# ml4ai/mliis

Hardware: AMD Instinct MI355X
Metric: inner-loop images/sec (EfficientLab-6-3, 224x224, 5-shot) (higher is better)
Workload: dtype f32 (the long-K decoder convs and their filter gradients with every operand split exactly into three bf16 terms on the matrix cores, 6 term products, f32 accumulate: fp32-equivalent products; everything else the fp32 instruction)

## Files before the change

include/mliis_hip.h:

```cpp
#ifndef MLIIS_HIP_H
#define MLIIS_HIP_H

#include <stddef.h>
#include <stdint.h>

#ifdef __cplusplus
extern "C" {
#endif

#ifndef __HIP__
typedef struct ihipStream_t* hipStream_t;
#endif

#if defined(__GNUC__) || defined(__clang__)
#pragma GCC visibility push(default)
#endif

#define MLIIS_OK 0
#define MLIIS_ERR_ARG (-1)
#define MLIIS_ERR_UNSUPPORTED (-2)
#define MLIIS_ERR_ALIGN (-3)
#define MLIIS_ERR_LAUNCH (-4)
#define MLIIS_ERR_WORKSPACE (-5)

// ... 76 lines not shown
int mliis_conv2d_fwd_bnin_ok(int Nimg, int H, int W, int Cin, int Cout);
int mliis_conv2d_fwd_bnin(const float* z, int ldz, const float* bn_part, int bn_nblk, float eps, float momentum, float* mean, float* rstd,
                          float* moving_mean, float* moving_var, const float* gamma, const float* beta, const float* img_scale,
                          const float* res, int ldr, float* a_out, int lda_out, const float* wt, float* y, int ldy, int Nimg, int H, int W,
                          int Cin, int Cout, float* stats_part, int stats_swish, int* stats_nblk, int precision, float fp8_act_scale,
                          const float* fp8_w_amax, int y_dtype, hipStream_t stream);
int mliis_transpose_weights(const float* src, float* dst, const int* desc, int ndesc, long long total_tiles, float* amax, hipStream_t stream);
int mliis_weight_shadows(const float* src, float* dst, const int* desc, int ndesc, long long total_tiles, float* amax, void* x3_images,
                         const long long* x3_desc, int x3_ndesc, int x3_blocks, hipStream_t stream);
int mliis_weight_shadows_rng(const float* src, float* dst, const int* desc, int ndesc, long long total_tiles, float* amax, void* x3_images,
                             const long long* x3_desc, int x3_ndesc, int x3_blocks, unsigned* rng_state, int njobs, float* const* outs,
                             const long long* numels, const float* keep, const float* const* keeps, const int* row_len, const int* floor_form,
                             hipStream_t stream);
int mliis_conv2d_bwd_data(const float* dy, int lddy, const float* w, float* dx, int lddx, int Nimg, int H, int W, int Cin_total,
                          int ci_begin, int Cin_out, int Cout, int ksize, int dil, int accumulate, float* ws, size_t ws_floats,
                          int precision, int dy_dtype, int dx_dtype, hipStream_t stream);
int mliis_conv2d_bwd_data_bn(const float* dy, int lddy, const float* w, float* dx, int lddx, int Nimg, int H, int W, int Cin_total,
                             int ci_begin, int Cin_out, int Cout, int ksize, int dil, int accumulate, float* ws, size_t ws_floats,
                             int precision, const float* bn_x, int bn_ldx, const float* bn_mean, const float* bn_rstd,
                             const float* bn_img_scale, float* part, size_t part_floats, int* nblk, int dy_dtype, int dx_dtype, hipStream_t stream);
int mliis_conv2d_bwd_data_gate(const float* dy, int lddy, const float* w, float* dx, int lddx, int Nimg, int H, int W, int Cin_total,
                               int ci_begin, int Cin_out, int Cout, int ksize, int dil, float* ws, size_t ws_floats, int precision,
                               const float* gate_x, int gate_ldx, float* part, size_t part_floats, int* groups, int dy_dtype, int dx_dtype, hipStream_t stream);
size_t mliis_x3_image_bytes(int Cred, int Nout, int ksize);
int mliis_x3_image_blocks(int Cred, int Nout, int ksize);
int mliis_x3_pack_weights(const float* theta, void* images, const long long* desc, int ndesc, int total_blocks, hipStream_t stream);
size_t mliis_conv2d_x3_workspace_floats(int Nimg, int H, int W, int Cred, int Nout, int ksize);
int mliis_conv2d_x3_plan(int Nimg, int H, int W, int Cred, int Nout, int ksize, int* plan);
int mliis_conv2d_fwd_x3(const float* x, int ldx, const void* image, size_t image_bytes, const float* bias, const float* border_bias, float* y, int ldy, int Nimg,
                        int H, int W, int Cin, int Cout, int ksize, int dil, int accumulate, float* stats_part, int stats_swish,
                        int* stats_nblk, float* ws, size_t ws_floats, hipStream_t stream);
int mliis_conv2d_bwd_data_x3(const float* dy, int lddy, const void* image, size_t image_bytes, float* dx, int lddx, int Nimg, int H, int W, int Cin_out, int Cout,
                             int ksize, int dil, int accumulate, float* ws, size_t ws_floats, hipStream_t stream);
size_t mliis_conv2d_bwd_filter_workspace_floats(int Nimg, int H, int W, int Cin, int Cout, int ksize);
int mliis_conv2d_bwd_filter(const float* x, int ldx, const float* x_scale, const float* dy, int lddy, float* dw, int Nimg, int H, int W,
                            int Cin_total, int ci_begin, int Cin, int Cout, int ksize, int dil, int accumulate, float* ws,
                            size_t ws_floats, int precision, hipStream_t stream);
int mliis_conv2d_bwd_filter_plan(int Nimg, int H, int W, int Cin, int Cout, int ksize, int* plan);
int mliis_conv2d_bwd_filter_batched(const long long* desc, int nprob, int blocks, int tmf, int nt, int has_scale, int precision,
                                    hipStream_t stream);

size_t mliis_rsd_concat_pool_floats(int N, int H, int W, int C);
int mliis_rsd_concat_pool(const float* deep, int ld_deep, int Hi, int Wi, int Cd, const float* skip, int ld_skip, int Cs, float* cat, int ldcat,
                          int N, int H, int W, float* pool_part, size_t pool_part_floats, int* chunks, hipStream_t stream);
int mliis_rsd_pool_fwd(const float* pool_part, int chunks, float scale, float* pool_out, const float* w, float* border_bias, int N, int Cp,
                       int Cin_total, int c_begin, int Co, hipStream_t stream);
// ... 111 lines not shown
```

mliis_amd/csrc/conv_gemm_kernels.hpp:

```cpp
#pragma once
#include <stdlib.h>

#include <type_traits>

#include "bn_fold.hpp"
#include "common.hpp"

namespace mliis {

typedef float f32x4 __attribute__((ext_vector_type(4)));

struct ConvGemmParams {
  const float* A;
  int lda;
  int Nimg, H, W;
  int C;
  int ntaps, dil, sign;
  const float* B;
  long long b_tap_stride;
  int ldb;
  int Nout;
  float* Cmat;
  int ldc;
  const float* bias;
// ... 1515 lines not shown
    case 5: L(T_, 5)  \
    case 6: L(T_, 6)  \
    case 7: L(T_, 7)  \
    default: L(T_, 8) \
  }
  if (f.tmf == 2) {
    ROW(2)
  } else {
    ROW(1)
  }
#undef ROW
#undef L
}

constexpr int kX3Block = 3072;
constexpr int kX3DescWords = 8;
__device__ __forceinline__ void x3_pack_block(const float* __restrict__ theta, char* __restrict__ images, const long long* __restrict__ desc,
                                              int ndesc, int b, int t) {
  int j = 0;
  for (int k = 1; k < ndesc; ++k)
    if (b >= (int)(desc[k * kX3DescWords + 6] >> 8)) j = k;
  const long long* d = desc + (long long)j * kX3DescWords;
  const float* w = theta + d[0];
  const int taps = (int)d[1], cin_total = (int)d[2], cout = (int)d[3], ci_begin = (int)d[4], cin = (int)d[5], mode = (int)(d[6] & 0xff);
  const int local = b - (int)(d[6] >> 8);
  const int nn = mode == 0 ? cout : cin, kc = mode == 0 ? cin : cout;
  const int ncol16 = (nn + 15) / 16;
  const int chunk = local / ncol16, c16 = local - chunk * ncol16;
  const int nl = t & 15, kq = t >> 4;
  const int n = c16 * 16 + nl;
  const int k = chunk * 32 + kq * 4;
  const int tap = k / kc, c = k - tap * kc;
  float4 v = f4zero();
  if (n < nn && tap < taps) {
    if (mode == 0) {
      const float* s = w + ((long long)tap * cin_total + ci_begin + c) * cout + n;
      v = make_float4(s[0], s[cout], s[2 * (long long)cout], s[3 * (long long)cout]);
    } else {
      v = ld4(w + ((long long)tap * cin_total + ci_begin + n) * cout + c);
    }
  }
  uint2 h, m, l;
  split3(v, h, m, l);
  char* dst = images + d[7] + (long long)local * kX3Block + (kq & 3) * 256 + nl * 16 + (kq >> 2) * 8;
  *reinterpret_cast<uint2*>(dst) = h;
  *reinterpret_cast<uint2*>(dst + 1024) = m;
  *reinterpret_cast<uint2*>(dst + 2048) = l;
}


void launch_gemm_bf16(const GemmPlan& g, const ConvGemmParams& p, hipStream_t stream);
void launch_gemm_sk_bf16(const GemmPlan& g, const ConvGemmParams& p, float* slab, hipStream_t stream);
void launch_gemm_fp8(const GemmPlan& g, const ConvGemmParams& p, hipStream_t stream);
bool launch_stream_lowp(int precision, int kc, int nt, dim3 grid, const ConvGemmParams& p, int row_groups, hipStream_t stream, bool ain = false);
bool launch_ksplit_lowp(int precision, int kc, int nt, dim3 grid, const ConvGemmParams& p, int row_groups, hipStream_t stream);
void launch_filter_bf16(const FilterPlan& f, const FilterGradParams& p, hipStream_t stream);
bool launch_filter_batched_bf16(int tmf, int nt, bool sc, const long long* desc, int nprob, int blocks, hipStream_t stream);
bool launch_filter_batched_x3(int nt, const long long* desc, int nprob, int blocks, int tile_ci, hipStream_t stream);

}
```

mliis_amd/csrc/conv_x3.hip:

```cpp
#include "conv_gemm_kernels.hpp"

namespace mliis {

constexpr int kX3BM = 256;
constexpr int kX3PF = 1;

__global__ __launch_bounds__(128) void x3_pack_k(const float* __restrict__ theta, char* __restrict__ images, const long long* __restrict__ desc,
                                                  int ndesc) {
  x3_pack_block(theta, images, desc, ndesc, blockIdx.x, threadIdx.x);
}

struct X3Params {
  ConvGemmParams g;
  const char* image;
  int ncol16;
};

template <int NT>
struct X3Sm {
  static constexpr int BN = 16 * NT;
  static constexpr int B_BYTES = NT * kX3Block;
  static constexpr int STAGES = 2;
  static constexpr int BYTES = STAGES * B_BYTES + 64;
};

template <int NT>
__device__ __forceinline__ void conv_x3_tile(const X3Params& q, char* __restrict__ sm, unsigned bx, int by, int it0, int it1,
                                             float* __restrict__ pdst) {
  constexpr int BN = 16 * NT;
  constexpr int B_BYTES = X3Sm<NT>::B_BYTES;
  constexpr int NB = (NT * 192 + 511) / 512;
  const ConvGemmParams& p = q.g;
  const int t = threadIdx.x, lane = t & 63;
  const int wave = __builtin_amdgcn_readfirstlane(t >> 6);
  const int l15 = lane & 15, g = lane >> 4;
  const long long M = (long long)p.Nimg * p.H * p.W;
  const long long m0 = (long long)bx * kX3BM;
  const int n0 = by * BN;
  const __amdgpu_buffer_rsrc_t rA = __builtin_amdgcn_make_buffer_rsrc((void*)p.A, 0, kBufRecords, 0x00020000);
  const __amdgpu_buffer_rsrc_t rB = __builtin_amdgcn_make_buffer_rsrc((void*)q.image, 0, kBufRecords, 0x00020000);

  const int wrow = wave * 32;
  unsigned a_row[2], a_taps[2];
#pragma unroll
  for (int rb = 0; rb < 2; ++rb) {
    const long long m = m0 + wrow + rb * 16 + l15;
    a_taps[rb] = 0;
    a_row[rb] = 0;
    if (m < M) {
      a_row[rb] = (unsigned)(m * p.lda * 4);
      if (p.ntaps > 1) {
        const int HWp = p.H * p.W;
        const int n = (int)(m / HWp);
        const int rem = (int)(m - (long long)n * HWp);
        const int h = rem / p.W, w_ = rem - h * p.W;
#pragma unroll
        for (int tp = 0; tp < 9; ++tp) {
          const int dh = (tp / 3 - 1) * p.dil * p.sign, dw = (tp % 3 - 1) * p.dil * p.sign;
          if ((unsigned)(h + dh) < (unsigned)p.H && (unsigned)(w_ + dw) < (unsigned)p.W) a_taps[rb] |= 1u << tp;
        }
      } else {
        a_taps[rb] = 1u;
      }
    }
  }
  int l_tap[2], l_c[2];
#pragma unroll
  for (int qd = 0; qd < 2; ++qd) {
    const int k0 = it0 * 32 + qd * 16 + g * 4;
    l_tap[qd] = k0 / p.C;
    l_c[qd] = k0 - l_tap[qd] * p.C;
  }
  int s_aleft = it1 - it0, s_bleft = it1 - it0;
  int ncol_here = q.ncol16 - by * NT;
  if (ncol_here > NT) ncol_here = NT;
  const unsigned b_lim = (unsigned)ncol_here * 192u;
  const unsigned b_step = (unsigned)q.ncol16 * kX3Block;
  unsigned b_voff[NB];
#pragma unroll
  for (int i = 0; i < NB; ++i) b_voff[i] = ((unsigned)t + 512u * i < b_lim) ? (unsigned)(by * NT) * kX3Block + ((unsigned)t + 512u * i) * 16u : kOob;
  unsigned s_boff = (unsigned)it0 * b_step;

  float4 ra[2][2];
  float4 ra2[2][2];
  u32x4 rbv[NB];
  const int tap_scale = p.dil * p.sign;
  auto load_a_into = [&](float4 (&ra)[2][2]) {
    const int adv = s_aleft > 1 ? 1 : 0;
    s_aleft -= adv;
#pragma unroll
    for (int qd = 0; qd < 2; ++qd) {
      const int tap = l_tap[qd];
      const int th = p.ntaps > 1 ? (tap * 11) >> 5 : 1, tw = p.ntaps > 1 ? tap - 3 * th : 1;
      const int dh = (th - 1) * tap_scale, dw = (tw - 1) * tap_scale;
      const unsigned koff = (unsigned)(((dh * p.W + dw) * p.lda + l_c[qd]) * 4);
      const unsigned tapbit = tap < p.ntaps ? 1u << tap : 0u;
#pragma unroll
      for (int rb = 0; rb < 2; ++rb) ra[rb][qd] = buf_ld4(rA, (a_taps[rb] & tapbit) != 0 ? a_row[rb] + koff : kOob);
      const int c_next = l_c[qd] + 32;
      const int wrap = c_next >= p.C ? 1 : 0;
      l_c[qd] = adv ? (wrap ? c_next - p.C : c_next) : l_c[qd];
      l_tap[qd] += adv & wrap;
    }
  };
  auto load_b_into = [&](u32x4 (&rbv)[NB]) {
#pragma unroll
    for (int i = 0; i < NB; ++i) {
      rbv[i] = __builtin_amdgcn_raw_buffer_load_b128(rB, (int)b_voff[i], (int)s_boff, 0);
    }
    const int adv = s_bleft > 1 ? 1 : 0;
    s_bleft -= adv;
    s_boff += adv ? b_step : 0u;
  };
  auto store_b_from = [&](char* buf, const u32x4 (&rbv)[NB]) {
#pragma unroll
    for (int i = 0; i < NB; ++i) {
      const int idx = t + 512 * i;
      char* d = (512 * (i + 1) <= NT * 192 || idx < NT * 192) ? buf + idx * 16 : sm + X3Sm<NT>::STAGES * B_BYTES + (t & 3) * 16;
      *reinterpret_cast<u32x4*>(d) = rbv[i];
// ... 79 lines not shown
      for (int rb = 0; rb < 2; ++rb) a3[pl][rb] = a3n[pl][rb];
  };
  {
    int it = 0;
    for (; it + 2 <= nper; it += 2) {
      chunk(sm, sm + B_BYTES, ra);
      chunk(sm + B_BYTES, sm, ra2);
    }
    if (it < nper) chunk(sm, sm + B_BYTES, ra);
  }
  asm volatile("s_waitcnt vmcnt(0)" ::: "memory");
#pragma unroll
  for (int rb = 0; rb < 2; ++rb)
#pragma unroll
    for (int r = 0; r < 4; ++r) {
      const int row = wrow + rb * 16 + g * 4 + r;
      if (m0 + row >= M) continue;
#pragma unroll
      for (int j = 0; j < NT; ++j)
        if (n0 + j * 16 + l15 < p.Nout) pdst[(long long)row * BN + j * 16 + l15] = acc[rb][j][r];
    }
}

template <int NT>
__global__ __launch_bounds__(512) void conv_x3_k(X3Params q, SkPlan k) {
  __shared__ __attribute__((aligned(16))) char sm[X3Sm<NT>::BYTES];
  constexpr int BN = 16 * NT;
#ifndef X3_NO_CLAIM
  asm volatile("v_mov_b32 v255, 0" ::: "v255");
#endif
  const int part = (int)xcd_remap(blockIdx.x, gridDim.x);
  int lo = part * k.ipp;
  const int total = k.rem * k.nchunks;
  int hi = lo + k.ipp;
  if (hi > total) hi = total;
#pragma unroll 1
  while (lo < hi) {
    const int rt = lo / k.nchunks, c0 = lo - rt * k.nchunks;
    int c1 = c0 + (hi - lo);
    if (c1 > k.nchunks) c1 = k.nchunks;
    const int first = (rt * k.nchunks) / k.ipp;
    float* dst = k.slab + ((long long)rt * k.smax + (part - first)) * (kX3BM * BN);
    conv_x3_tile<NT>(q, sm, rt / k.gy, rt % k.gy, c0, c1, dst);
    lo += c1 - c0;
    __syncthreads();
  }
}

constexpr int kX3Fix = 4;
template <int NT>
__global__ __launch_bounds__(1024) void x3_fixup_k(ConvGemmParams p, SkPlan k) {
  constexpr int BN = 16 * NT, QN = BN / 4;
  constexpr int QS = QN <= 32 ? 32 : 64;
  constexpr int RL = 1024 / QS;
  constexpr int RPT = kX3BM / kX3Fix / RL;
  __shared__ float4 red[2][RL][QS];
  const int t = threadIdx.x, q = t % QS, rl = t / QS;
  const int rt = blockIdx.x, sub = blockIdx.y;
  const unsigned tau = k.full + rt;
  const int bx = tau / k.gy, by = tau % k.gy;
  const long long M = (long long)p.Nimg * p.H * p.W;
  const int r0 = sub * (kX3BM / kX3Fix);
  const long long m0 = (long long)bx * kX3BM + r0;
  const int n = by * BN + q * 4;
  const bool cok = q < QN && n < p.Nout;
  const int first = (rt * k.nchunks) / k.ipp;
  int last = ((rt + 1) * k.nchunks - 1) / k.ipp;
  if (last > k.parts - 1) last = k.parts - 1;
  const int nslots = last - first + 1;
// ... 316 lines not shown
struct X3Plan {
  int nt, gx, gy, nchunks;
  int full, rem, parts, ipp, smax;
  size_t slab_floats() const { return (size_t)rem * smax * kX3BM * (16 * nt); }
};
constexpr int kX3MinPart = 4;

constexpr int kX3MaxNT = 9;
static int x3_pick_nt(int Nout) {
  int best = 1;
  double best_cost = 1e30;
  const int tiles = (Nout + 15) / 16;
  for (int nt = 1; nt <= kX3MaxNT; ++nt) {
    const int blocks = (tiles + nt - 1) / nt;
    const double cost = (double)(blocks * nt * 16) / (double)Nout * (1.0 + 0.08 * (8 - nt));
    if (cost < best_cost - 1e-9 || (cost < best_cost + 1e-9 && nt > best)) {
      best_cost = cost;
      best = nt;
    }
  }
  return best;
}

static inline int x3_chunks(int ntaps, int Cred) { return (ntaps * Cred + 31) / 32; }
static X3Plan x3_plan(long long M, int Nout, int ntaps, int Cred, int num_cus) {
  X3Plan g;
  g.nt = x3_pick_nt(Nout);
  g.gy = (Nout + g.nt * 16 - 1) / (g.nt * 16);
  g.gx = (int)((M + kX3BM - 1) / kX3BM);
  g.nchunks = x3_chunks(ntaps, Cred);
  const int slots = num_cus;
  while (g.nt > 2 && (long long)g.gx * g.gy * g.nchunks < (long long)slots * 2 * kX3MinPart) {
    g.nt = (g.nt + 1) / 2;
    g.gy = (Nout + g.nt * 16 - 1) / (g.nt * 16);
  }
  const long long tiles = (long long)g.gx * g.gy;
  g.full = 0;
  g.rem = (int)tiles;
  const long long total = tiles * g.nchunks;
  long long parts = slots;
  if (parts > 8LL * tiles) parts = 8LL * tiles;
  if (total / parts < kX3MinPart) parts = total / kX3MinPart;
  if (parts < 1) parts = 1;
  g.ipp = (int)((total + parts - 1) / parts);
  g.parts = (int)((total + g.ipp - 1) / g.ipp);
  g.smax = (g.nchunks + g.ipp - 1) / g.ipp + 1;
  return g;
}

static int g_x3_cus = 0;
static int x3_num_cus() {
  if (g_x3_cus == 0) {
    int dev = 0;
    hipDeviceProp_t prop;
    g_x3_cus = (hipGetDevice(&dev) == hipSuccess && hipGetDeviceProperties(&prop, dev) == hipSuccess && prop.multiProcessorCount > 0)
                   ? prop.multiProcessorCount
                   : 256;
  }
  return g_x3_cus;
}

static void x3_launch(const X3Plan& g, const X3Params& q_, float* slab, hipStream_t stream) {
  X3Params q = q_;
  const SkPlan k{g.full, g.rem, g.parts, g.ipp, g.nchunks, g.smax, g.gy, slab};
  dim3 grid(g.parts), block(512);
#define L(NT_)                                                                                  \
  hipLaunchKernelGGL((conv_x3_k<NT_>), grid, block, 0, stream, q, k);                           \
  hipLaunchKernelGGL((x3_fixup_k<NT_>), dim3(g.rem, kX3Fix), dim3(1024), 0, stream, q.g, k);    \
  break;
  switch (g.nt) {
    case 1: L(1)
    case 2: L(2)
    case 3: L(3)
    case 4: L(4)
    case 5: L(5)
    case 6: L(6)
    case 7: L(7)
    case 8: L(8)
    default: L(9)
  }
#undef L
}

static int x3_shape_check(const char* name, int Nimg, int H, int W, int Cred, int Nout, int ksize, int dil) {
  MLIIS_REQUIRE(Nimg > 0 && H > 0 && W > 0 && Cred >= 32 && Nout > 0, MLIIS_ERR_ARG, "%s: bad shape (the reduced channel count must be >= 32)", name);
  MLIIS_REQUIRE((Cred & 3) == 0 && (Nout & 3) == 0, MLIIS_ERR_ARG, "%s: channel counts must be multiples of 4", name);
  MLIIS_REQUIRE(ksize == 1 || ksize == 3, MLIIS_ERR_UNSUPPORTED, "%s: kernel size %d unsupported (1 or 3)", name, ksize);
  MLIIS_REQUIRE(dil >= 1, MLIIS_ERR_ARG, "%s: dilation must be >= 1", name);
  return MLIIS_OK;
}

}

using namespace mliis;

extern "C" {

size_t mliis_x3_image_bytes(int Cred, int Nout, int ksize) {
  return (size_t)x3_chunks(ksize * ksize, Cred) * ((Nout + 15) / 16) * kX3Block;
}

int mliis_x3_image_blocks(int Cred, int Nout, int ksize) { return x3_chunks(ksize * ksize, Cred) * ((Nout + 15) / 16); }

int mliis_x3_pack_weights(const float* theta, void* images, const long long* desc, int ndesc, int total_blocks, hipStream_t stream) {
  MLIIS_REQUIRE(theta && images && desc && ndesc >= 1 && ndesc <= 64 && total_blocks >= 1, MLIIS_ERR_ARG, "x3_pack_weights: bad arguments");
  MLIIS_REQUIRE(aligned16(theta) && aligned16(images) && aligned16(desc), MLIIS_ERR_ALIGN, "x3_pack_weights: pointers must be 16-byte aligned");
  hipLaunchKernelGGL(x3_pack_k, dim3(total_blocks), dim3(128), 0, stream, theta, reinterpret_cast<char*>(images), desc, ndesc);
  MLIIS_CHECK_LAUNCH("x3_pack_weights");
  return MLIIS_OK;
}

size_t mliis_conv2d_x3_workspace_floats(int Nimg, int H, int W, int Cred, int Nout, int ksize) {
  return x3_plan((long long)Nimg * H * W, Nout, ksize * ksize, Cred, x3_num_cus()).slab_floats();
}

int mliis_conv2d_x3_plan(int Nimg, int H, int W, int Cred, int Nout, int ksize, int* plan) {
  MLIIS_REQUIRE(plan, MLIIS_ERR_ARG, "conv2d_x3_plan: null pointer");
  const X3Plan g = x3_plan((long long)Nimg * H * W, Nout, ksize * ksize, Cred, x3_num_cus());
  plan[0] = g.nt; plan[1] = g.gx; plan[2] = g.gy; plan[3] = g.full; plan[4] = g.parts; plan[5] = g.ipp;
  return MLIIS_OK;
}

int mliis_conv2d_fwd_x3(const float* x, int ldx, const void* image, size_t image_bytes, const float* bias, const float* border_bias, float* y, int ldy, int Nimg,
                        int H, int W, int Cin, int Cout, int ksize, int dil, int accumulate, float* stats_part, int stats_swish,
                        int* stats_nblk, float* ws, size_t ws_floats, hipStream_t stream) {
  int rc = x3_shape_check("conv2d_fwd_x3", Nimg, H, W, Cin, Cout, ksize, dil);
  if (rc) return rc;
  MLIIS_REQUIRE(x && image && y, MLIIS_ERR_ARG, "conv2d_fwd_x3: null pointer");
  MLIIS_REQUIRE(image_bytes == mliis_x3_image_bytes(Cin, Cout, ksize), MLIIS_ERR_ARG,
                "conv2d_fwd_x3: the weight image has %zu bytes, a forward image over %d reduced channels x %d columns (k = %d) has %zu -- packed for another "
                "window or direction?", image_bytes, Cin, Cout, ksize, mliis_x3_image_bytes(Cin, Cout, ksize));
  MLIIS_REQUIRE((ldx & 3) == 0 && ldx >= Cin && (ldy & 3) == 0 && ldy >= Cout, MLIIS_ERR_ARG, "conv2d_fwd_x3: bad leading dimensions");
  MLIIS_REQUIRE(aligned16(x) && aligned16(image) && aligned16(bias) && aligned16(y) && aligned16(border_bias) && aligned16(ws), MLIIS_ERR_ALIGN,
                "conv2d_fwd_x3: pointers must be 16-byte aligned");
  const long long M = (long long)Nimg * H * W;
  MLIIS_REQUIRE(M * ldx * 4 < (1LL << 31) && mliis_x3_image_bytes(Cin, Cout, ksize) < (1ULL << 31), MLIIS_ERR_UNSUPPORTED,
                "conv2d_fwd_x3: operand larger than 2 GiB (32-bit buffer offsets)");
  MLIIS_REQUIRE(border_bias == nullptr || (ksize == 3 && dil == 1 && H >= 2 && W >= 2), MLIIS_ERR_ARG,
                "conv2d_fwd_x3: border_bias needs a 3x3 dilation-1 conv on a map of at least 2x2");
  MLIIS_REQUIRE(stats_part == nullptr || (!accumulate && stats_nblk), MLIIS_ERR_ARG,
                "conv2d_fwd_x3: fused statistics need accumulate == 0 and a stats_nblk output");
  const X3Plan g = x3_plan(M, Cout, ksize * ksize, Cin, x3_num_cus());
  MLIIS_REQUIRE(g.slab_floats() == 0 || (ws != nullptr && g.slab_floats() <= ws_floats), MLIIS_ERR_WORKSPACE,
                "conv2d_fwd_x3: workspace too small (%zu needed, %zu given)", g.slab_floats(), ws_floats);
  X3Params q{};
  q.g = ConvGemmParams{x, ldx, Nimg, H, W, Cin, ksize * ksize, dil, +1, nullptr, 0, 0, Cout, y, ldy, bias, accumulate, nullptr, 0,
                       stats_part, stats_swish, nullptr, border_bias, 1.0f, nullptr};
  q.image = reinterpret_cast<const char*>(image);
  q.ncol16 = (Cout + 15) / 16;
  x3_launch(g, q, ws, stream);
  MLIIS_CHECK_LAUNCH("conv2d_fwd_x3");
  if (stats_nblk) *stats_nblk = stats_part != nullptr ? g.gx * kX3Fix : 0;
  return MLIIS_OK;
}

int mliis_conv2d_bwd_data_x3(const float* dy, int lddy, const void* image, size_t image_bytes, float* dx, int lddx, int Nimg, int H, int W, int Cin_out, int Cout,
                             int ksize, int dil, int accumulate, float* ws, size_t ws_floats, hipStream_t stream) {
  int rc = x3_shape_check("conv2d_bwd_data_x3", Nimg, H, W, Cout, Cin_out, ksize, dil);
  if (rc) return rc;
  MLIIS_REQUIRE(dy && image && dx, MLIIS_ERR_ARG, "conv2d_bwd_data_x3: null pointer");
  MLIIS_REQUIRE(image_bytes == mliis_x3_image_bytes(Cout, Cin_out, ksize), MLIIS_ERR_ARG,
                "conv2d_bwd_data_x3: the weight image has %zu bytes, a backward-data image over %d reduced channels x %d columns (k = %d) has %zu -- packed "
                "for another window or direction?", image_bytes, Cout, Cin_out, ksize, mliis_x3_image_bytes(Cout, Cin_out, ksize));
  MLIIS_REQUIRE((lddy & 3) == 0 && lddy >= Cout && (lddx & 3) == 0 && lddx >= Cin_out, MLIIS_ERR_ARG, "conv2d_bwd_data_x3: bad leading dimensions");
  MLIIS_REQUIRE(aligned16(dy) && aligned16(image) && aligned16(dx) && aligned16(ws), MLIIS_ERR_ALIGN,
                "conv2d_bwd_data_x3: pointers must be 16-byte aligned");
  const long long M = (long long)Nimg * H * W;
  MLIIS_REQUIRE(M * lddy * 4 < (1LL << 31) && mliis_x3_image_bytes(Cout, Cin_out, ksize) < (1ULL << 31), MLIIS_ERR_UNSUPPORTED,
                "conv2d_bwd_data_x3: operand larger than 2 GiB (32-bit buffer offsets)");
  const X3Plan g = x3_plan(M, Cin_out, ksize * ksize, Cout, x3_num_cus());
  MLIIS_REQUIRE(g.slab_floats() == 0 || (ws != nullptr && g.slab_floats() <= ws_floats), MLIIS_ERR_WORKSPACE,
                "conv2d_bwd_data_x3: workspace too small (%zu needed, %zu given)", g.slab_floats(), ws_floats);
  X3Params q{};
  q.g = ConvGemmParams{dy, lddy, Nimg, H, W, Cout, ksize * ksize, dil, -1, nullptr, 0, 0, Cin_out, dx, lddx, nullptr, accumulate, nullptr, 0,
                       nullptr, 0, nullptr, nullptr, 1.0f, nullptr};
  q.image = reinterpret_cast<const char*>(image);
  q.ncol16 = (Cin_out + 15) / 16;
  x3_launch(g, q, ws, stream);
  MLIIS_CHECK_LAUNCH("conv2d_bwd_data_x3");
  return MLIIS_OK;
}
}
```

mliis_amd/learner.py:

```python
from __future__ import annotations

import ctypes as C
import functools
import os
from typing import Dict, List, Optional, Sequence

import numpy as np
import torch

from . import ops, spec
from ._lib import MliisError, lib
from .arena import Arena
from .passes import _Passes
from .plan import _Plan


class Learner(_Passes):
    def __init__(self, feature_extractor_name: str = "efficientnet-b0", image_size: int = 224, rsd: Optional[Sequence[int]] = (2, 4),
                 learning_rate: float = 1e-3, optimizer: str = "sgd", l2: bool = False, l1: bool = False, darc1: bool = False,
                 dice: bool = False, label_smoothing: float = 0.0, final_layer_dropout_rate: float = 0.0,
                 spatial_pyramid_pooling: bool = False, skip_decoding: bool = False, drop_connect: bool = True, seed: int = 0,
                 device="cuda:0", use_graph: bool = True, max_shots: int = 16, matmul_precision: str = "fp32",
                 small_fused: Optional[bool] = None, dw_march: Optional[bool] = None, fuse_bn2: Optional[bool] = None, fuse_head: Optional[bool] = None,
                 augment_batch_capacity: int = 0, rng_stream: int = 0):
# ... 73 lines not shown
            self._aug_ops_dev = torch.zeros(8 * self.aug_capacity * 48, dtype=torch.uint8, device=self.device)
            self._aug_ops_pin = torch.zeros((4, 8 * self.aug_capacity * 48), dtype=torch.uint8).pin_memory()
            self._aug_ev = [None] * 4
            self._aug_n = 0
        self.n_shots = 0
        self._aug_valid = 0
        self.rng_state = ops.rng_state((int(seed) & 0xFFFFFFFF) ^ ((int(rng_stream) & 0xFFFFFFFF) << 32) if rng_stream else seed, self.device)
        self._dc_keeps = torch.tensor([1.0 - b.drop_rate for b in self.arch.executed() if b.skip] or [1.0], dtype=torch.float32, device=self.device)
        self.drop_keep_dev = torch.tensor([1.0 - self.final_layer_dropout_rate], dtype=torch.float32, device=self.device)
        self._drop_keep_val = 1.0 - self.final_layer_dropout_rate
        self._rng_now = None
        self._pname()
        self.x3 = None
        if self.x3_on:
            self.x3 = ops.X3Images(self.device)
            shapes = {p.name: p.shape for p in A.trainable}
            for m, nm in zip(self.arch.rsd, self.n_rsd):
                (k0, _, _), (k1, _, _), (kf, _, _) = nm
                for name, cin in ((k1, None), (kf, 2 * m.c_out)):
                    kk, _, cin_total, cout = shapes[name]
                    win = cin_total if cin is None else cin
                    if ops.X3Images.eligible(win, cout, kk) and ops.X3Images.eligible(cout, win, kk):
                        self.x3.add(name, "fwd", A.t_off[name], kk, cin_total, cout, 0, win)
                        self.x3.add(name, "bwd", A.t_off[name], kk, cin_total, cout, 0, win)
            self.x3.finish()
        torch.cuda.synchronize(self.device)

    def _pname(self):
        fe = self.arch.name
        self.n_stem = (f"{fe}/stem/conv2d/kernel", f"{fe}/stem/tpu_batch_normalization")
        self.n_blocks = []
        for b in self.arch.executed():
            s = f"{fe}/blocks_{b.idx}"
            bns = [f"{s}/tpu_batch_normalization", f"{s}/tpu_batch_normalization_1", f"{s}/tpu_batch_normalization_2"]
            cvs = [f"{s}/conv2d/kernel", f"{s}/conv2d_1/kernel"]
            d = {}
            if b.expand != 1:
                d["w_exp"], d["bn0"] = cvs.pop(0), bns.pop(0)
            d["w_dw"], d["bn1"] = f"{s}/depthwise_conv2d/depthwise_kernel", bns.pop(0)
            d["se"] = (f"{s}/se/conv2d/kernel", f"{s}/se/conv2d/bias", f"{s}/se/conv2d_1/kernel", f"{s}/se/conv2d_1/bias")
            d["w_proj"], d["bn2"] = cvs.pop(0), bns.pop(0)
            self.n_blocks.append(d)
        self.n_rsd, self.n_rsd_up = [], []
        for m in self.arch.rsd:
            s = f"decode/decode_skip_connections_{m.scope_index}"
            sfx = ["", "_1", "_2", "_3"]
            trip = lambda x: (f"{s}/conv2d{x}/kernel", f"{s}/conv2d{x}/bias", f"{s}/batch_normalization{x}")
# ... 394 lines not shown
```

mliis_amd/ops.py:

```python
from __future__ import annotations

import ctypes as C
import os
from typing import Optional, Tuple

import torch

from ._lib import MliisError, lib, score_lib
from .spec import BN_EPS, BN_MOMENTUM, MEAN_RGB, STDDEV_RGB

_MEAN3 = (C.c_float * 3)(*MEAN_RGB)
_STD3 = (C.c_float * 3)(*STDDEV_RGB)


def _stream() -> int:
    return torch.cuda.current_stream().cuda_stream


def _ptr(t: Optional[torch.Tensor]):
    if t is None:
        return None
    if not t.is_cuda:
        raise MliisError("mliis_amd ops need device tensors (no CPU path)")
    if t.dtype == torch.bfloat16:
# ... 451 lines not shown
        raise MliisError("conv2d_fwd_bnin: stats_part too small")
    meta = _conv_meta(N, H, W, Cin, Cout, 1, 1, precision=precision, splits=1)
    nb = C.c_int(0)
    _timed("conv2d_fwd", meta, lambda: lib.call("mliis_conv2d_fwd_bnin", _ptr(_chk(z)), ldz, _ptr(part), int(nblk), eps, momentum, _ptr(mean), _ptr(rstd),
                                                _ptr(mm), _ptr(mv), _ptr(gamma), _ptr(beta), _ptr(img_scale), _ptr(res), ldr, _ptr(a_out), ldo,
                                                _ptr(wt), _aptr(out), ldy, N, H, W, Cin, Cout, _ptr(stats_part), int(stats_swish), C.byref(nb), prec,
                                                float(fp8_act_scale), _ptr(fp8_w_amax), _dt(out) | (int(out_block) << 8), _stream()))
    return out, nb.value


class X3Images:

    X3_MIN_K = 512

    def __init__(self, device):
        self.device = device
        self.rows, self.view, self.blocks, self.bytes = [], {}, 0, 0
        self.images = self.desc = None

    @staticmethod
    def eligible(cred, nout, k) -> bool:
        return cred >= 32 and cred % 4 == 0 and nout % 4 == 0 and k * k * cred >= X3Images.X3_MIN_K

    def add(self, key, mode, theta_off, k, cin_total, cout, ci_begin=0, cin=None):
        cin = cin_total - ci_begin if cin is None else cin
        cred, nout = (cin, cout) if mode == "fwd" else (cout, cin)
        nbytes = lib.size("mliis_x3_image_bytes", cred, nout, k)
        nblk = lib.size("mliis_x3_image_blocks", cred, nout, k)
        self.rows.append([int(theta_off), k * k, cin_total, cout, ci_begin, cin, (0 if mode == "fwd" else 1) | (self.blocks << 8), self.bytes])
        self.view[(key, mode)] = (self.bytes, nbytes)
        self.blocks += nblk
        self.bytes += nbytes

    def finish(self):
        self.images = torch.zeros(max(self.bytes, 16), dtype=torch.uint8, device=self.device)
        self.desc = torch.tensor(self.rows, dtype=torch.int64, device=self.device) if self.rows else None
        return self

    def pack(self, theta):
        if self.desc is not None:
            lib.call("mliis_x3_pack_weights", _ptr(theta), _ptr(self.images), _ptr(self.desc), len(self.rows), self.blocks, _stream())

    def image(self, key, mode):
        off, n = self.view[(key, mode)]
        return self.images[off:off + n]

    def has(self, key, mode):
        return (key, mode) in self.view


def x3_image_of(w, mode, ci_begin=0, cin=None):
    k, _, cin_total, cout = w.shape
    im = X3Images(w.device)
    im.add("w", mode, 0, k, cin_total, cout, ci_begin, cin)
    im.finish().pack(w.contiguous().view(-1))
    return im.image("w", mode)


def conv2d_x3_kernel_name(N, H, W, cred, nout, k):
    plan = (C.c_int * 8)()
    lib.call("mliis_conv2d_x3_plan", N, H, W, cred, nout, k, plan)
    return "conv_x3_k<%d>" % plan[0]


def conv2d_fwd_x3(x, image, k, cout, bias=None, dil=1, out=None, accumulate=False, ws: Optional[Workspace] = None, stats_part=None,
                  stats_swish=False, border_bias=None):
    N, H, W = x.shape[:3]
    rows, Cin, ldx = rows_ld(x)
    _dense(image, bias, border_bias, stats_part)
    _out_rows(out, (N, H, W, cout), what="conv2d_fwd_x3 out")
    out = torch.empty((N, H, W, cout), dtype=torch.float32, device=x.device) if out is None else out
    _, co, ldy = rows_ld(out)
    ws = ws or default_ws()
    buf = ws.get(lib.size("mliis_conv2d_x3_workspace_floats", N, H, W, Cin, cout, k))
    nblk = C.c_int(0)
    meta = _conv_meta(N, H, W, Cin, cout, k, dil, x3=True)
    _timed("conv2d_fwd_x3", meta, lambda: lib.call("mliis_conv2d_fwd_x3", _aptr(x), ldx, _ptr(image), image.numel() * image.element_size(), _ptr(bias), _ptr(border_bias), _aptr(out), ldy,
                                                   N, H, W, Cin, cout, k, dil, int(accumulate), _ptr(stats_part), int(stats_swish), C.byref(nblk),
                                                   _ptr(buf), buf.numel(), _stream()))
    if stats_part is not None:
        return out, nblk.value
    return out


def conv2d_bwd_data_x3(dy, image, k, cin_out, dil=1, out=None, accumulate=False, ws: Optional[Workspace] = None):
    N, H, W = dy.shape[:3]
    rows, Cout, lddy = rows_ld(dy)
    _dense(image)
    _out_rows(out, (N, H, W, cin_out), what="conv2d_bwd_data_x3 out")
    out = torch.empty((N, H, W, cin_out), dtype=torch.float32, device=dy.device) if out is None else out
    _, ci, lddx = rows_ld(out)
    ws = ws or default_ws()
    buf = ws.get(lib.size("mliis_conv2d_x3_workspace_floats", N, H, W, Cout, cin_out, k))
    meta = _conv_meta(N, H, W, Cout, cin_out, k, dil, x3=True)
    _timed("conv2d_bwd_data_x3", meta, lambda: lib.call("mliis_conv2d_bwd_data_x3", _aptr(dy), lddy, _ptr(image), image.numel() * image.element_size(), _aptr(out), lddx, N, H, W, cin_out,
                                                        Cout, k, dil, int(accumulate), _ptr(buf), buf.numel(), _stream()))
    return out


def conv1x1_stream_eligible(N, H, W, cred, nout, precision="fp32"):
    return conv2d_kernel_name(N, H, W, cred, nout, 1, False, precision).startswith("conv1x1_stream_k")


def conv2d_bwd_data(dy, w, dil=1, ci_begin=0, ci_count=None, out=None, accumulate=False, ws: Optional[Workspace] = None, precision="fp32",
                    bn=None, part=None, gate=None, out_block=0):
    N, H, W = dy.shape[:3]
    k, _, Cin, Cout = w.shape
    ci_count = Cin - ci_begin if ci_count is None else ci_count
    _, cy, lddy = rows_ld(dy)
    if cy != Cout:
        raise MliisError("conv2d_bwd_data: dy has {} channels, weight has {}".format(cy, Cout))
    _dense(w, part, *((bn[1], bn[2], bn[3]) if bn is not None else ()))
    if not out_block:
        _out_rows(out, (N, H, W, ci_count), None, what="conv2d_bwd_data out")
    out = torch.empty((N, H, W, ci_count), dtype=torch.float32, device=dy.device) if out is None else out
    _, _, lddx = rows_ld(out)
    ws = ws or default_ws()
    buf = ws.get(lib.size("mliis_conv2d_workspace_floats", N, H, W, Cout, ci_count, k))
    prec = _prec(precision)
# ... 599 lines not shown
```

mliis_amd/passes.py:

```python
from __future__ import annotations

import torch

from . import ops, spec
from ._lib import MliisError
from .plan import _Plan


class _Pass:

    def __init__(self, L, P: _Plan, training: bool, stochastic: bool = True):
        self.L, self.P, self.training = L, P, training
        self.stochastic = training and stochastic
        self.w, self.mv, self.g, self.ws = L.arena.w, L.arena.mv, L.arena.g, L.ws

    def moving(self, prefix):
        return self.mv[prefix + "/moving_mean"], self.mv[prefix + "/moving_variance"]

    def bn_bwd_args(self, st, prefix):
        return st[0], st[1], self.w[prefix + "/gamma"], self.w[prefix + "/beta"]

    def bn_fwd_args(self, st, prefix, moving=True):
        return (self.w[prefix + "/gamma"], self.w[prefix + "/beta"], st[0], st[1]) + (self.moving(prefix) if moving else (None, None))

# ... 343 lines not shown
        return P.blocks[bi]["dout"], tgt_has

    def _rsd_bwd(self, S: _Pass, j, has_grad):
        a, P, w, g, ws = self.arch, S.P, S.w, S.g, S.ws
        m, D, nm = a.rsd[j], P.rsd[j], self.n_rsd[j]
        (k0, b0, n0), (k1, b1, n1), (kf, bf, nf) = nm
        co = m.c_out
        dO, cat, pyr, dpyr, dcat = D["dout"], D["cat"], D["pyr"], D["dpyr"], D["dcat"]
        S.bn_b(D["zf"], dO, D["stf"], nf, D["dzf"], pre=True)
        ops.rsd_pool_bwd(D["dzf"], D["tot"], D["pool"], w[kf], 2 * co, dw=g[kf], dbias=g[bf], dpool=D["dpool"], ws=ws)
        S.wgrad_conv(pyr, D["dzf"], 3, 1, kf)
        S.conv_bwd_data(D["dzf"], kf, 1, 2 * co, dpyr)
        d0, d1 = dpyr[..., :co], dpyr[..., co:2 * co]
        ops.bn_bwd_pair([(D["z" + i], d_, *S.bn_bwd_args(D["st" + i], nn), d_, g[nn + "/gamma"], g[nn + "/beta"], P.fold_part[bb])
                         for i, d_, nn, bb in (("0", d0, n0, b0), ("1", d1, n1, b1))], pre_swish=True, ws=ws)
        tail = P.filter_tail[j]
        cmain = cat[..., :m.c_cat - tail] if tail else cat

        def wgrad(dz, kname, kk, dil, cmain=cmain, ctail=cat[..., m.c_cat - tail:] if tail else None):
            S.wgrad_conv(cmain, dz, kk, dil, kname)
            if ctail is not None:
                S.wgrad_conv(ctail, dz, kk, dil, kname + "#tail")
        wgrad(d0, k0, 1, 1)
        self._conv_bwd_data(d0, w[k0], 1, out=dcat, ws=ws)
        wgrad(d1, k1, 3, 2)
        S.conv_bwd_data(d1, k1, 2, m.c_cat, dcat, accumulate=True)
        bi_skip = a.reductions[m.scope_index + 1]
        if m.upsample_conv:
            ku, bu, nu = self.n_rsd_up[j]
            S.bn_b(D["zu"], dO, D["stu"], nu, D["dzu"], pre=True, dxsum_part=P.fold_part[bu])
            S.wgrad_conv(cat[..., :m.c_deep], D["dzu"], 1, 1, ku)
            self._conv_bwd_data(D["dzu"], w[ku], 1, out=D["dup"], ws=ws)
            dU = D["dup"]
        else:
            dU = dO
        ops.chan_split(dcat, m.c_deep, dU, True, P.blocks[bi_skip]["dout"], has_grad[bi_skip], A=D["dpool"])
        has_grad[bi_skip] = True
        tgt, tgt_has = self._deep_grad_target(P, has_grad, j)
        if m.h_in == m.h:
            ops.chan_affine(dU, out=tgt, accumulate=tgt_has)
        else:
            ops.resize_bilinear_bwd(dU, (m.h_in, m.h_in), out=tgt, accumulate=tgt_has)

    def _skipdec_bwd(self, S: _Pass, has_grad):
        a, P, w, ws = self.arch, S.P, S.w, S.ws
        sd, T = a.skipdec, P.skipdec
        (k0, n0), seps = self.n_skipdec
        d = T["dout"]
        for Q, (dwn, dbn, pwn, pbn) in zip(reversed(T["sep"]), reversed(seps)):
# ... 107 lines not shown
```

Baseline: 3591.

## Fuse 1x1 backward-data into 3x3 x3 backward-data as an extra rider tap

The 1x1 conv's backward-data is folded into the dilated 3x3 conv's split-bf16 backward-data GEMM. The 1x1 weights are packed as a tenth tap of the weight image, and the A operand reads the adjacent dy channel slice for that tap. This removes a separate kernel launch, a write of dcat followed by an accumulate read-modify-write, and gives the 1x1 product fp32-equivalent matrix-core precision. In exchange it lengthens the K reduction, which can change the split-K plan, and it requires d0 and d1 to be adjacent slices in one buffer.

```diff
diff --git a/include/mliis_hip.h b/include/mliis_hip.h
--- a/include/mliis_hip.h
+++ b/include/mliis_hip.h
@@ -122,6 +122,7 @@
 int mliis_conv2d_bwd_data_gate(const float* dy, int lddy, const float* w, float* dx, int lddx, int Nimg, int H, int W, int Cin_total,
                                int ci_begin, int Cin_out, int Cout, int ksize, int dil, float* ws, size_t ws_floats, int precision,
                                const float* gate_x, int gate_ldx, float* part, size_t part_floats, int* groups, int dy_dtype, int dx_dtype, hipStream_t stream);
+#define MLIIS_X3_RIDER 0x100
 size_t mliis_x3_image_bytes(int Cred, int Nout, int ksize);
 int mliis_x3_image_blocks(int Cred, int Nout, int ksize);
 int mliis_x3_pack_weights(const float* theta, void* images, const long long* desc, int ndesc, int total_blocks, hipStream_t stream);
diff --git a/mliis_amd/csrc/conv_gemm_kernels.hpp b/mliis_amd/csrc/conv_gemm_kernels.hpp
--- a/mliis_amd/csrc/conv_gemm_kernels.hpp
+++ b/mliis_amd/csrc/conv_gemm_kernels.hpp
@@ -1561,7 +1561,8 @@
     if (b >= (int)(desc[k * kX3DescWords + 6] >> 8)) j = k;
   const long long* d = desc + (long long)j * kX3DescWords;
   const float* w = theta + d[0];
-  const int taps = (int)d[1], cin_total = (int)d[2], cout = (int)d[3], ci_begin = (int)d[4], cin = (int)d[5], mode = (int)(d[6] & 0xff);
+  const int taps = (int)(d[1] & 0xff), cin_total = (int)d[2], cout = (int)d[3], ci_begin = (int)d[4], cin = (int)d[5], mode = (int)(d[6] & 0xff);
+  const long long src2 = d[1] >> 8;
   const int local = b - (int)(d[6] >> 8);
   const int nn = mode == 0 ? cout : cin, kc = mode == 0 ? cin : cout;
   const int ncol16 = (nn + 15) / 16;
@@ -1578,6 +1579,8 @@
     } else {
       v = ld4(w + ((long long)tap * cin_total + ci_begin + n) * cout + c);
     }
+  } else if (n < nn && tap == taps && src2 != 0) {
+    v = ld4(theta + (src2 - 1) + ((long long)ci_begin + n) * cout + c);
   }
   uint2 h, m, l;
   split3(v, h, m, l);
diff --git a/mliis_amd/csrc/conv_x3.hip b/mliis_amd/csrc/conv_x3.hip
--- a/mliis_amd/csrc/conv_x3.hip
+++ b/mliis_amd/csrc/conv_x3.hip
@@ -14,6 +14,7 @@
   ConvGemmParams g;
   const char* image;
   int ncol16;
+  int tap_coff, extra_coff;
 };
 
 template <int NT>
@@ -24,7 +25,7 @@
   static constexpr int BYTES = STAGES * B_BYTES + 64;
 };
 
-template <int NT>
+template <int NT, bool EXTRA = false>
 __device__ __forceinline__ void conv_x3_tile(const X3Params& q, char* __restrict__ sm, unsigned bx, int by, int it0, int it1,
                                              float* __restrict__ pdst) {
   constexpr int BN = 16 * NT;
@@ -62,6 +63,7 @@
       } else {
         a_taps[rb] = 1u;
       }
+      if (EXTRA) a_taps[rb] |= 1u << 9;
     }
   }
   int l_tap[2], l_c[2];
@@ -92,9 +94,11 @@
     for (int qd = 0; qd < 2; ++qd) {
       const int tap = l_tap[qd];
       const int th = p.ntaps > 1 ? (tap * 11) >> 5 : 1, tw = p.ntaps > 1 ? tap - 3 * th : 1;
-      const int dh = (th - 1) * tap_scale, dw = (tw - 1) * tap_scale;
-      const unsigned koff = (unsigned)(((dh * p.W + dw) * p.lda + l_c[qd]) * 4);
-      const unsigned tapbit = tap < p.ntaps ? 1u << tap : 0u;
+      const bool ex = EXTRA && tap >= 9;
+      const int dh = ex ? 0 : (th - 1) * tap_scale, dw = ex ? 0 : (tw - 1) * tap_scale;
+      const int coff = EXTRA ? (ex ? q.extra_coff : q.tap_coff) : 0;
+      const unsigned koff = (unsigned)(((dh * p.W + dw) * p.lda + l_c[qd] + coff) * 4);
+      const unsigned tapbit = tap < (EXTRA ? 10 : p.ntaps) ? 1u << tap : 0u;
 #pragma unroll
       for (int rb = 0; rb < 2; ++rb) ra[rb][qd] = buf_ld4(rA, (a_taps[rb] & tapbit) != 0 ? a_row[rb] + koff : kOob);
       const int c_next = l_c[qd] + 32;
@@ -220,9 +224,8 @@
     }
 }
 
-template <int NT>
-__global__ __launch_bounds__(512) void conv_x3_k(X3Params q, SkPlan k) {
-  __shared__ __attribute__((aligned(16))) char sm[X3Sm<NT>::BYTES];
+template <int NT, bool EXTRA>
+__device__ __forceinline__ void conv_x3_parts(const X3Params& q, const SkPlan& k, char* __restrict__ sm) {
   constexpr int BN = 16 * NT;
 #ifndef X3_NO_CLAIM
   asm volatile("v_mov_b32 v255, 0" ::: "v255");
@@ -239,10 +242,20 @@
     if (c1 > k.nchunks) c1 = k.nchunks;
     const int first = (rt * k.nchunks) / k.ipp;
     float* dst = k.slab + ((long long)rt * k.smax + (part - first)) * (kX3BM * BN);
-    conv_x3_tile<NT>(q, sm, rt / k.gy, rt % k.gy, c0, c1, dst);
+    conv_x3_tile<NT, EXTRA>(q, sm, rt / k.gy, rt % k.gy, c0, c1, dst);
     lo += c1 - c0;
     __syncthreads();
   }
+}
+template <int NT>
+__global__ __launch_bounds__(512) void conv_x3_k(X3Params q, SkPlan k) {
+  __shared__ __attribute__((aligned(16))) char sm[X3Sm<NT>::BYTES];
+  conv_x3_parts<NT, false>(q, k, sm);
+}
+template <int NT>
+__global__ __launch_bounds__(512) void conv_x3_cat_k(X3Params q, SkPlan k) {
+  __shared__ __attribute__((aligned(16))) char sm[X3Sm<NT>::BYTES];
+  conv_x3_parts<NT, true>(q, k, sm);
 }
 
 constexpr int kX3Fix = 4;
@@ -605,6 +618,9 @@
   return best;
 }
 
+static inline int x3_ksize(int ksize) { return ksize & 0xff; }
+static inline bool x3_rider(int ksize) { return (ksize & MLIIS_X3_RIDER) != 0; }
+static inline int x3_taps(int ksize) { return x3_ksize(ksize) * x3_ksize(ksize) + (x3_rider(ksize) ? 1 : 0); }
 static inline int x3_chunks(int ntaps, int Cred) { return (ntaps * Cred + 31) / 32; }
 static X3Plan x3_plan(long long M, int Nout, int ntaps, int Cred, int num_cus) {
   X3Plan g;
@@ -643,12 +659,13 @@
   return g_x3_cus;
 }
 
-static void x3_launch(const X3Plan& g, const X3Params& q_, float* slab, hipStream_t stream) {
+static void x3_launch(const X3Plan& g, const X3Params& q_, float* slab, hipStream_t stream, bool extra = false) {
   X3Params q = q_;
   const SkPlan k{g.full, g.rem, g.parts, g.ipp, g.nchunks, g.smax, g.gy, slab};
   dim3 grid(g.parts), block(512);
 #define L(NT_)                                                                                  \
-  hipLaunchKernelGGL((conv_x3_k<NT_>), grid, block, 0, stream, q, k);                           \
+  if (extra) hipLaunchKernelGGL((conv_x3_cat_k<NT_>), grid, block, 0, stream, q, k);            \
+  else hipLaunchKernelGGL((conv_x3_k<NT_>), grid, block, 0, stream, q, k);                      \
   hipLaunchKernelGGL((x3_fixup_k<NT_>), dim3(g.rem, kX3Fix), dim3(1024), 0, stream, q.g, k);    \
   break;
   switch (g.nt) {
@@ -665,7 +682,10 @@
 #undef L
 }
 
-static int x3_shape_check(const char* name, int Nimg, int H, int W, int Cred, int Nout, int ksize, int dil) {
+static int x3_shape_check(const char* name, int Nimg, int H, int W, int Cred, int Nout, int ksize_flags, int dil, bool rider_ok = false) {
+  const int ksize = x3_ksize(ksize_flags);
+  MLIIS_REQUIRE((ksize_flags & ~(0xff | MLIIS_X3_RIDER)) == 0 && (!x3_rider(ksize_flags) || (rider_ok && ksize == 3)), MLIIS_ERR_ARG,
+                "%s: MLIIS_X3_RIDER goes with the backward-data of a 3x3 conv only (ksize argument 0x%x)", name, ksize_flags);
   MLIIS_REQUIRE(Nimg > 0 && H > 0 && W > 0 && Cred >= 32 && Nout > 0, MLIIS_ERR_ARG, "%s: bad shape (the reduced channel count must be >= 32)", name);
   MLIIS_REQUIRE((Cred & 3) == 0 && (Nout & 3) == 0, MLIIS_ERR_ARG, "%s: channel counts must be multiples of 4", name);
   MLIIS_REQUIRE(ksize == 1 || ksize == 3, MLIIS_ERR_UNSUPPORTED, "%s: kernel size %d unsupported (1 or 3)", name, ksize);
@@ -680,10 +700,10 @@
 extern "C" {
 
 size_t mliis_x3_image_bytes(int Cred, int Nout, int ksize) {
-  return (size_t)x3_chunks(ksize * ksize, Cred) * ((Nout + 15) / 16) * kX3Block;
-}
-
-int mliis_x3_image_blocks(int Cred, int Nout, int ksize) { return x3_chunks(ksize * ksize, Cred) * ((Nout + 15) / 16); }
+  return (size_t)x3_chunks(x3_taps(ksize), Cred) * ((Nout + 15) / 16) * kX3Block;
+}
+
+int mliis_x3_image_blocks(int Cred, int Nout, int ksize) { return x3_chunks(x3_taps(ksize), Cred) * ((Nout + 15) / 16); }
 
 int mliis_x3_pack_weights(const float* theta, void* images, const long long* desc, int ndesc, int total_blocks, hipStream_t stream) {
   MLIIS_REQUIRE(theta && images && desc && ndesc >= 1 && ndesc <= 64 && total_blocks >= 1, MLIIS_ERR_ARG, "x3_pack_weights: bad arguments");
@@ -694,12 +714,12 @@
 }
 
 size_t mliis_conv2d_x3_workspace_floats(int Nimg, int H, int W, int Cred, int Nout, int ksize) {
-  return x3_plan((long long)Nimg * H * W, Nout, ksize * ksize, Cred, x3_num_cus()).slab_floats();
+  return x3_plan((long long)Nimg * H * W, Nout, x3_taps(ksize), Cred, x3_num_cus()).slab_floats();
 }
 
 int mliis_conv2d_x3_plan(int Nimg, int H, int W, int Cred, int Nout, int ksize, int* plan) {
   MLIIS_REQUIRE(plan, MLIIS_ERR_ARG, "conv2d_x3_plan: null pointer");
-  const X3Plan g = x3_plan((long long)Nimg * H * W, Nout, ksize * ksize, Cred, x3_num_cus());
+  const X3Plan g = x3_plan((long long)Nimg * H * W, Nout, x3_taps(ksize), Cred, x3_num_cus());
   plan[0] = g.nt; plan[1] = g.gx; plan[2] = g.gy; plan[3] = g.full; plan[4] = g.parts; plan[5] = g.ipp;
   return MLIIS_OK;
 }
@@ -739,8 +759,10 @@
 
 int mliis_conv2d_bwd_data_x3(const float* dy, int lddy, const void* image, size_t image_bytes, float* dx, int lddx, int Nimg, int H, int W, int Cin_out, int Cout,
                              int ksize, int dil, int accumulate, float* ws, size_t ws_floats, hipStream_t stream) {
-  int rc = x3_shape_check("conv2d_bwd_data_x3", Nimg, H, W, Cout, Cin_out, ksize, dil);
+  int rc = x3_shape_check("conv2d_bwd_data_x3", Nimg, H, W, Cout, Cin_out, ksize, dil, true);
   if (rc) return rc;
+  const bool rider = x3_rider(ksize);
+  MLIIS_REQUIRE(!rider || lddy >= 2 * Cout, MLIIS_ERR_ARG, "conv2d_bwd_data_x3: MLIIS_X3_RIDER needs the %d channels below dy in the same rows (lddy %d)", Cout, lddy);
   MLIIS_REQUIRE(dy && image && dx, MLIIS_ERR_ARG, "conv2d_bwd_data_x3: null pointer");
   MLIIS_REQUIRE(image_bytes == mliis_x3_image_bytes(Cout, Cin_out, ksize), MLIIS_ERR_ARG,
                 "conv2d_bwd_data_x3: the weight image has %zu bytes, a backward-data image over %d reduced channels x %d columns (k = %d) has %zu -- packed "
@@ -749,17 +771,19 @@
   MLIIS_REQUIRE(aligned16(dy) && aligned16(image) && aligned16(dx) && aligned16(ws), MLIIS_ERR_ALIGN,
                 "conv2d_bwd_data_x3: pointers must be 16-byte aligned");
   const long long M = (long long)Nimg * H * W;
-  MLIIS_REQUIRE(M * lddy * 4 < (1LL << 31) && mliis_x3_image_bytes(Cout, Cin_out, ksize) < (1ULL << 31), MLIIS_ERR_UNSUPPORTED,
+  MLIIS_REQUIRE((M * lddy + (rider ? Cout : 0)) * 4 < (1LL << 31) && mliis_x3_image_bytes(Cout, Cin_out, ksize) < (1ULL << 31), MLIIS_ERR_UNSUPPORTED,
                 "conv2d_bwd_data_x3: operand larger than 2 GiB (32-bit buffer offsets)");
-  const X3Plan g = x3_plan(M, Cin_out, ksize * ksize, Cout, x3_num_cus());
+  const X3Plan g = x3_plan(M, Cin_out, x3_taps(ksize), Cout, x3_num_cus());
   MLIIS_REQUIRE(g.slab_floats() == 0 || (ws != nullptr && g.slab_floats() <= ws_floats), MLIIS_ERR_WORKSPACE,
                 "conv2d_bwd_data_x3: workspace too small (%zu needed, %zu given)", g.slab_floats(), ws_floats);
   X3Params q{};
-  q.g = ConvGemmParams{dy, lddy, Nimg, H, W, Cout, ksize * ksize, dil, -1, nullptr, 0, 0, Cin_out, dx, lddx, nullptr, accumulate, nullptr, 0,
-                       nullptr, 0, nullptr, nullptr, 1.0f, nullptr};
+  q.g = ConvGemmParams{rider ? dy - Cout : dy, lddy, Nimg, H, W, Cout, x3_ksize(ksize) * x3_ksize(ksize), dil, -1, nullptr, 0, 0, Cin_out, dx, lddx, nullptr,
+                       accumulate, nullptr, 0, nullptr, 0, nullptr, nullptr, 1.0f, nullptr};
   q.image = reinterpret_cast<const char*>(image);
   q.ncol16 = (Cin_out + 15) / 16;
-  x3_launch(g, q, ws, stream);
+  q.tap_coff = rider ? Cout : 0;
+  q.extra_coff = 0;
+  x3_launch(g, q, ws, stream, rider);
   MLIIS_CHECK_LAUNCH("conv2d_bwd_data_x3");
   return MLIIS_OK;
 }
diff --git a/mliis_amd/learner.py b/mliis_amd/learner.py
--- a/mliis_amd/learner.py
+++ b/mliis_amd/learner.py
@@ -119,7 +119,10 @@
                     win = cin_total if cin is None else cin
                     if ops.X3Images.eligible(win, cout, kk) and ops.X3Images.eligible(cout, win, kk):
                         self.x3.add(name, "fwd", A.t_off[name], kk, cin_total, cout, 0, win)
-                        self.x3.add(name, "bwd", A.t_off[name], kk, cin_total, cout, 0, win)
+                        if name == k1 and tuple(shapes[k0]) == (1, 1, cin_total, cout):
+                            self.x3.add(name, "bwdcat", A.t_off[name], kk, cin_total, cout, 0, win, extra_off=A.t_off[k0])
+                        else:
+                            self.x3.add(name, "bwd", A.t_off[name], kk, cin_total, cout, 0, win)
             self.x3.finish()
         torch.cuda.synchronize(self.device)
 
diff --git a/mliis_amd/ops.py b/mliis_amd/ops.py
--- a/mliis_amd/ops.py
+++ b/mliis_amd/ops.py
@@ -497,12 +497,20 @@
     def eligible(cred, nout, k) -> bool:
         return cred >= 32 and cred % 4 == 0 and nout % 4 == 0 and k * k * cred >= X3Images.X3_MIN_K
 
-    def add(self, key, mode, theta_off, k, cin_total, cout, ci_begin=0, cin=None):
+    def add(self, key, mode, theta_off, k, cin_total, cout, ci_begin=0, cin=None, extra_off=None):
         cin = cin_total - ci_begin if cin is None else cin
         cred, nout = (cin, cout) if mode == "fwd" else (cout, cin)
-        nbytes = lib.size("mliis_x3_image_bytes", cred, nout, k)
-        nblk = lib.size("mliis_x3_image_blocks", cred, nout, k)
-        self.rows.append([int(theta_off), k * k, cin_total, cout, ci_begin, cin, (0 if mode == "fwd" else 1) | (self.blocks << 8), self.bytes])
+        if (mode == "bwdcat") != (extra_off is not None):
+            raise MliisError("X3Images.add: extra_off goes with mode \"bwdcat\" and only with it")
+        taps, src2 = k * k, 0
+        if mode == "bwdcat":
+            nbytes = lib.size("mliis_x3_image_bytes", cred, nout, k | X3_RIDER)
+            nblk = lib.size("mliis_x3_image_blocks", cred, nout, k | X3_RIDER)
+            src2 = (int(extra_off) + 1) << 8
+        else:
+            nbytes = lib.size("mliis_x3_image_bytes", cred, nout, k)
+            nblk = lib.size("mliis_x3_image_blocks", cred, nout, k)
+        self.rows.append([int(theta_off), taps | src2, cin_total, cout, ci_begin, cin, (0 if mode == "fwd" else 1) | (self.blocks << 8), self.bytes])
         self.view[(key, mode)] = (self.bytes, nbytes)
         self.blocks += nblk
         self.bytes += nbytes
@@ -530,6 +538,17 @@
     im.add("w", mode, 0, k, cin_total, cout, ci_begin, cin)
     im.finish().pack(w.contiguous().view(-1))
     return im.image("w", mode)
+
+
+def x3_image_cat_of(w, w1, ci_begin=0, cin=None):
+    k, _, cin_total, cout = w.shape
+    if tuple(w1.shape) != (1, 1, cin_total, cout):
+        raise MliisError("x3_image_cat_of: the 1x1 weights must be [1,1,{},{}], got {}".format(cin_total, cout, tuple(w1.shape)))
+    theta = torch.cat([w.contiguous().view(-1), w1.contiguous().view(-1)])
+    im = X3Images(w.device)
+    im.add("w", "bwdcat", 0, k, cin_total, cout, ci_begin, cin, extra_off=w.numel())
+    im.finish().pack(theta)
+    return im.image("w", "bwdcat")
 
 
 def conv2d_x3_kernel_name(N, H, W, cred, nout, k):
@@ -570,6 +589,35 @@
     meta = _conv_meta(N, H, W, Cout, cin_out, k, dil, x3=True)
     _timed("conv2d_bwd_data_x3", meta, lambda: lib.call("mliis_conv2d_bwd_data_x3", _aptr(dy), lddy, _ptr(image), image.numel() * image.element_size(), _aptr(out), lddx, N, H, W, cin_out,
                                                         Cout, k, dil, int(accumulate), _ptr(buf), buf.numel(), _stream()))
+    return out
+
+
+X3_RIDER = 0x100
+
+
+def conv2d_bwd_data_x3_cat(dy, dy1, image, k, cin_out, dil=1, out=None, accumulate=False, ws: Optional[Workspace] = None):
+    N, H, W = dy.shape[:3]
+    rows, Cout, lddy = rows_ld(dy)
+    rows1, Cout1, lddy1 = rows_ld(dy1)
+    if (tuple(dy1.shape) != tuple(dy.shape) or lddy1 != lddy or dy.dtype != torch.float32 or dy1.dtype != torch.float32
+            or dy1.untyped_storage().data_ptr() != dy.untyped_storage().data_ptr() or dy.data_ptr() - dy1.data_ptr() != 4 * Cout
+            or lddy < 2 * Cout):
+        raise MliisError("conv2d_bwd_data_x3_cat: dy1 must be the channel slice just below dy in the same rows of one fp32 buffer; got shapes "
+                         "{} / {}, strides {} / {}, offsets {} / {}".format(tuple(dy.shape), tuple(dy1.shape), dy.stride(), dy1.stride(),
+                                                                            dy.storage_offset(), dy1.storage_offset()))
+    _dense(image)
+    _out_rows(out, (N, H, W, cin_out), what="conv2d_bwd_data_x3_cat out")
+    out = torch.empty((N, H, W, cin_out), dtype=torch.float32, device=dy.device) if out is None else out
+    _, ci, lddx = rows_ld(out)
+    ws = ws or default_ws()
+    buf = ws.get(lib.size("mliis_conv2d_x3_workspace_floats", N, H, W, Cout, cin_out, k | X3_RIDER))
+    meta = {}
+    if PROFILE is not None:
+        plan = (C.c_int * 8)()
+        lib.call("mliis_conv2d_x3_plan", N, H, W, Cout, cin_out, k | X3_RIDER, plan)
+        meta = dict(kernel="conv_x3_cat_k<%d>" % plan[0], flops=2.0 * N * H * W * (k * k + 1) * cin_out * Cout, shape=(N, H, W, cin_out, Cout, k, dil))
+    _timed("conv2d_bwd_data_x3_cat", meta, lambda: lib.call("mliis_conv2d_bwd_data_x3", _aptr(dy), lddy, _ptr(image), image.numel() * image.element_size(), _aptr(out),
+                                                            lddx, N, H, W, cin_out, Cout, k | X3_RIDER, dil, int(accumulate), _ptr(buf), buf.numel(), _stream()))
     return out
 
 
diff --git a/mliis_amd/passes.py b/mliis_amd/passes.py
--- a/mliis_amd/passes.py
+++ b/mliis_amd/passes.py
@@ -389,9 +389,12 @@
             if ctail is not None:
                 S.wgrad_conv(ctail, dz, kk, dil, kname + "#tail")
         wgrad(d0, k0, 1, 1)
-        self._conv_bwd_data(d0, w[k0], 1, out=dcat, ws=ws)
         wgrad(d1, k1, 3, 2)
-        S.conv_bwd_data(d1, k1, 2, m.c_cat, dcat, accumulate=True)
+        if self._x3_takes(k1, d1) and self.x3.has(k1, "bwdcat"):
+            ops.conv2d_bwd_data_x3_cat(d1, d0, self.x3.image(k1, "bwdcat"), 3, m.c_cat, 2, out=dcat, ws=ws)
+        else:
+            self._conv_bwd_data(d0, w[k0], 1, out=dcat, ws=ws)
+            S.conv_bwd_data(d1, k1, 2, m.c_cat, dcat, accumulate=True)
         bi_skip = a.reductions[m.scope_index + 1]
         if m.upsample_conv:
             ku, bu, nu = self.n_rsd_up[j]
```

After: 3627, median of 6. Within noise of the previous version (+1.0%).
